# spartan-array/spartan

Measured on AMD Instinct MI355X. Metric: spartan.dot TFLOP/s (+ map/reduce HBM GB/s), higher is better.
Workload: dtype f32

## Files before the change

### spartan_amd/csrc/gemm_split.hpp

```cpp
#pragma once

typedef __bf16 gs_bf16x8 __attribute__((ext_vector_type(8)));
typedef __bf16 gs_bf16x4 __attribute__((ext_vector_type(4)));

namespace {

constexpr int GS_BK = 16;
constexpr int GS_RB = GS_BK * 2;
constexpr int GS_WN = 4;
constexpr unsigned GS_WIN_LO = (127u - 40u) << 23;
constexpr unsigned GS_WIN_HI = (127u + 40u) << 23;
constexpr size_t GS_IMAGE_CAP = (size_t)2 << 30;
constexpr size_t GS_WS_HEAD = 512;

template <int WN>
struct GsCfg {
  static constexpr int BM = 256, BN = 64 * WN, NW = 2 * WN, THREADS = 64 * NW;
  static constexpr int A_BYTES = BM * GS_RB, B_BYTES = BN * GS_RB;
  static constexpr int STAGE_BYTES = 3 * A_BYTES + 3 * B_BYTES;
  static constexpr int SMEM_BYTES = 2 * STAGE_BYTES;
  static constexpr int APW = A_BYTES / 1024 / NW, BPW = B_BYTES / 1024 / NW;
  static constexpr int NPIECES = 3 * APW + 3 * BPW;
  static constexpr int SLOTS = SP_CUS * (WN == 4 ? 1 : 2);
  static_assert(APW >= 1 && BPW >= 1 && APW * NW * 1024 == A_BYTES && BPW * NW * 1024 == B_BYTES, "tile / waves mismatch");
  static_assert(NPIECES * 4 <= 48, "one piece after every fourth MFMA");
};

__device__ __forceinline__ bool gs_outside(float v) {
  const unsigned b = __float_as_uint(v) & 0x7fffffffu;
  return b != 0u && (b < GS_WIN_LO || b >= GS_WIN_HI);
}

__device__ __forceinline__ void gs_cut(float v, __bf16& h, __bf16& m, __bf16& l) {
  h = (__bf16)v;
  const float r1 = v - (float)h;
  m = (__bf16)r1;
  l = (__bf16)(r1 - (float)m);
}

__device__ __forceinline__ void gs_raise(bool bad, unsigned* flag) {
  if (__any(bad) && (threadIdx.x & 63) == 0) atomicOr(flag, 1u);
}

__global__ __launch_bounds__(256) void sp_gemm_cut_rows_kernel(const float* __restrict__ A, int64_t lda, int M, int K,
                                                               __bf16* __restrict__ Ah, int64_t img,
                                                               unsigned* __restrict__ flag) {
  const int q = threadIdx.x & 7, row = blockIdx.x * 32 + (threadIdx.x >> 3);
  const int kpad = (K + GS_BK - 1) / GS_BK * GS_BK;
  bool bad = false;
  if (row < M) {
    const float* __restrict__ a = A + (int64_t)row * lda;
#pragma unroll
    for (int it = 0; it < 8; ++it) {
      const int k = blockIdx.y * 256 + it * 32 + 4 * q;
      if (k >= kpad) break;
      f32x4 v = {0.f, 0.f, 0.f, 0.f};
      if (k + 4 <= K) {
        v = *(const f32x4*)(a + k);
      } else {
#pragma unroll
        for (int e = 0; e < 4; ++e)
          if (k + e < K) v[e] = a[k + e];
      }
      gs_bf16x4 h, m, l;
#pragma unroll
      for (int e = 0; e < 4; ++e) {
        bad |= gs_outside(v[e]);
        __bf16 hh, mm, ll;
        gs_cut(v[e], hh, mm, ll);
        h[e] = hh;
        m[e] = mm;
        l[e] = ll;
      }
      const int64_t at = ((int64_t)(k >> 4) * M + row) * GS_BK + (k & 15);
      *(gs_bf16x4*)(Ah + at) = h;
      *(gs_bf16x4*)(Ah + img + at) = m;
      *(gs_bf16x4*)(Ah + 2 * img + at) = l;
    }
  }
  gs_raise(bad, flag);
}

__global__ __launch_bounds__(256) void sp_gemm_cut_cols_kernel(const float* __restrict__ B, int64_t ldb, int N, int K,
                                                               __bf16* __restrict__ Bh, int64_t img,
                                                               unsigned* __restrict__ flag) {
  __shared__ __attribute__((aligned(16))) __bf16 s[3][256 * GS_BK];
  const int n0 = blockIdx.x * 256, col = n0 + threadIdx.x, k0 = blockIdx.y * GS_BK;
  float v[GS_BK];
#pragma unroll
  for (int e = 0; e < GS_BK; ++e) v[e] = (col < N && k0 + e < K) ? B[(int64_t)(k0 + e) * ldb + col] : 0.f;
  bool bad = false;
  gs_bf16x8 h[2], m[2], l[2];
#pragma unroll
  for (int e = 0; e < GS_BK; ++e) {
    bad |= gs_outside(v[e]);
    __bf16 hh, mm, ll;
    gs_cut(v[e], hh, mm, ll);
    h[e >> 3][e & 7] = hh;
    m[e >> 3][e & 7] = mm;
    l[e >> 3][e & 7] = ll;
  }
#pragma unroll
  for (int c = 0; c < 2; ++c) {
    *(gs_bf16x8*)(&s[0][threadIdx.x * GS_BK + 8 * c]) = h[c];
    *(gs_bf16x8*)(&s[1][threadIdx.x * GS_BK + 8 * c]) = m[c];
    *(gs_bf16x8*)(&s[2][threadIdx.x * GS_BK + 8 * c]) = l[c];
  }
  __syncthreads();
  const int64_t base = ((int64_t)blockIdx.y * N + n0) * GS_BK;
#pragma unroll
  for (int p = 0; p < 3; ++p)
#pragma unroll
    for (int c = 0; c < 2; ++c) {
      const int at = (c * 256 + threadIdx.x) * 8;
      if (n0 + at / GS_BK < N) *(gs_bf16x8*)(Bh + p * img + base + at) = *(const gs_bf16x8*)(&s[p][at]);
    }
  gs_raise(bad, flag);
}

template <int WN>
__global__ __launch_bounds__(GsCfg<WN>::THREADS, 2) void sp_gemm_glds_kernel_bf16x3(
    const char* __restrict__ Ah, int64_t a_img, const char* __restrict__ Bh, int64_t b_img, float* __restrict__ C,
    int64_t ldc, int M, int N, int KT, int accumulate, int tiles_m, int tiles_n, int64_t a_slab, int64_t b_slab,
    const unsigned* __restrict__ flag_a, const unsigned* __restrict__ flag_b) {
  using G = GsCfg<WN>;
  constexpr int APW = G::APW, BPW = G::BPW, NPIECES = G::NPIECES;
  extern __shared__ __attribute__((aligned(16))) char gs_smem[];
  if ((*flag_a | *flag_b) != 0u) return;
  int tm, tn;
  sp_gemm_tile_of_block(blockIdx.x, gridDim.x, tiles_m, tiles_n, tm, tn);
  const int m0 = tm * G::BM, n0 = tn * G::BN;
  const int tid = threadIdx.x, lane = tid & 63;
  const int wid = __builtin_amdgcn_readfirstlane(tid >> 6);
  const int wm = wid / WN, wn = wid % WN;
  const int l31 = lane & 31, lh = lane >> 5;

  unsigned a_off[APW], b_off[BPW];
#pragma unroll
  for (int j = 0; j < APW; ++j) {
    const int slot = (wid * APW + j) * 64 + lane;
    int row = slot >> 1;
    const int q = (slot & 1) ^ ((row >> 4) & 1);
    if (m0 + row > M - 1) row = M - 1 - m0;
    a_off[j] = (unsigned)(row * GS_RB + q * 16);
  }
#pragma unroll
  for (int j = 0; j < BPW; ++j) {
    const int slot = (wid * BPW + j) * 64 + lane;
    int row = slot >> 1;
    const int q = (slot & 1) ^ ((row >> 4) & 1);
    if (n0 + row > N - 1) row = N - 1 - n0;
    b_off[j] = (unsigned)(row * GS_RB + q * 16);
  }
  const char* __restrict__ Ablk = Ah + (int64_t)m0 * GS_RB;
  const char* __restrict__ Bblk = Bh + (int64_t)n0 * GS_RB;
  const unsigned s_base = SP_LDS_ADDR(gs_smem);

#define GS_PIECE(i)                                                                                    \
  do {                                                                                                 \
    if ((i) < 3 * APW) {                                                                               \
      const int p_ = (i) / APW, j_ = (i) % APW;                                                        \
      SP_GLDS_S(Ablk + p_ * a_img + ka_, a_off[j_], st_ + p_ * G::A_BYTES + (wid * APW + j_) * 1024);  \
    } else {                                                                                           \
      const int p_ = ((i) - 3 * APW) / BPW, j_ = ((i) - 3 * APW) % BPW;                                \
      SP_GLDS_S(Bblk + p_ * b_img + kb_, b_off[j_],                                                    \
                st_ + 3 * G::A_BYTES + p_ * G::B_BYTES + (wid * BPW + j_) * 1024);                     \
    }                                                                                                  \
  } while (0)

  f32x16 acc[4][2];
#pragma unroll
  for (int i = 0; i < 4; ++i)
#pragma unroll
    for (int j = 0; j < 2; ++j)
#pragma unroll
      for (int r = 0; r < 16; ++r) acc[i][j][r] = 0.f;

  {
    const int64_t ka_ = 0, kb_ = 0;
    const unsigned st_ = s_base;
#pragma unroll
    for (int i = 0; i < NPIECES; ++i) GS_PIECE(i);
  }
  SP_GLDS_LANDED();
  __syncthreads();

  const int fslot = (lh ^ ((l31 >> 4) & 1)) * 16;
  const int a_frag = (wm * 128 + l31) * GS_RB + fslot;
  const int b_frag = 3 * G::A_BYTES + (wn * 64 + l31) * GS_RB + fslot;

  for (int t = 0; t < KT; ++t) {
    const bool more = t + 1 < KT;
    const int64_t ka_ = (int64_t)(t + 1) * a_slab, kb_ = (int64_t)(t + 1) * b_slab;
    const unsigned st_ = s_base + (unsigned)((t + 1) & 1) * G::STAGE_BYTES;
    const char* st = gs_smem + (t & 1) * G::STAGE_BYTES;
    gs_bf16x8 af[3][4], bf[3][2];
#pragma unroll
    for (int p = 0; p < 3; ++p) {
#pragma unroll
      for (int i = 0; i < 4; ++i) af[p][i] = *(const gs_bf16x8*)(st + p * G::A_BYTES + a_frag + i * 32 * GS_RB);
#pragma unroll
      for (int j = 0; j < 2; ++j) bf[p][j] = *(const gs_bf16x8*)(st + p * G::B_BYTES + b_frag + j * 32 * GS_RB);
    }
    int piece = 0;
#pragma unroll
    for (int idx = 0; idx < 48; ++idx) {
      const int term = idx >> 3, i = (idx & 7) >> 1, j = idx & 1;
      const int pa = term == 0 ? 2 : (term == 2 || term == 3) ? 1 : 0;
      const int pb = term == 1 ? 2 : (term == 2 || term == 4) ? 1 : 0;
      acc[i][j] = __builtin_amdgcn_mfma_f32_32x32x16_bf16(af[pa][i], bf[pb][j], acc[i][j], 0, 0, 0);
      if (idx % 4 == 3 && piece < NPIECES) {
        __builtin_amdgcn_sched_barrier(0);
        if (more) GS_PIECE(piece);
        __builtin_amdgcn_sched_barrier(0);
        ++piece;
      }
    }
    if (more) SP_GLDS_LANDED();
    __syncthreads();
  }
#undef GS_PIECE

#pragma unroll
  for (int i = 0; i < 4; ++i) {
#pragma unroll
    for (int j = 0; j < 2; ++j) {
      const int col = n0 + wn * 64 + j * 32 + l31;
#pragma unroll
      for (int r = 0; r < 16; ++r) {
        const int row = m0 + wm * 128 + i * 32 + (r & 3) + 8 * (r >> 2) + 4 * lh;
        if (row < M && col < N) {
          float* p = C + (int64_t)row * ldc + col;
          float v = acc[i][j][r];
          if (accumulate) v += *p;
          *p = v;
        }
      }
    }
  }
}

template <typename Cfg, int BM, int BN, int WM, int WN, int WGS>
__global__ __launch_bounds__(Cfg::THREADS, WGS) void sp_gemm_f32_gated_kernel(
    const float* __restrict__ A, int64_t lda, const float* __restrict__ B, int64_t ldb, float* __restrict__ C,
    int64_t ldc, int M, int N, int K, int accumulate, int tiles_m, int tiles_n, const unsigned* __restrict__ flag_a,
    const unsigned* __restrict__ flag_b) {
  if ((*flag_a | *flag_b) == 0u) return;
  sp_gemm_glds_body<Cfg, BM, BN, WM, WN>(A, lda, B, ldb, C, ldc, M, N, K, accumulate, tiles_m, tiles_n);
}

#define GS_CUT_BYTES_PER_S 3.0e12
#define GS_ISSUED_FLOPS 1.1e15
static bool sp_gemm_bf16_plan(int64_t M, int64_t N, int64_t K) {
  static int mode = -2;
  if (mode == -2) {
    const char* e = getenv("SP_GEMM_SPLIT");
    mode = e ? atoi(e) : 1;
  }
  using G = GsCfg<GS_WN>;
  if (mode == 0 || K < 16 || N % 4 != 0 || N < 4 || M < 1 || M > 2147483647LL || N > 2147483647LL || K > 2147483647LL)
    return false;
  const int64_t tb = ((M + 255) / 256) * ((N + 127) / 128);
  if (tb < 2 * SP_CUS || tb >= 2147483647LL) return false;
  double dp_cost;
  if (sp_gemm_dp_choice(M, N, &dp_cost) != 6 || sp_sk_plan(M, N, K)) return false;
  const int64_t KT = (K + GS_BK - 1) / GS_BK;
  if ((double)KT * 3.0 * GS_RB * ((double)M + (double)N) > (double)GS_IMAGE_CAP) return false;
  const double fp32_s = dp_cost * 128.0 * 128.0 * (double)K * 2.0 / (157.3e12 * 0.95 / SP_CUS);
  const int64_t tiles = ((M + G::BM - 1) / G::BM) * ((N + G::BN - 1) / G::BN);
  const int64_t rounds = (tiles + G::SLOTS - 1) / G::SLOTS;
  const double main_s = (double)rounds * G::SLOTS * (6.0 * 2.0 * G::BM * G::BN * (double)K) / GS_ISSUED_FLOPS;
  const double cut_s = 10.0 * ((double)M + (double)N) * (double)K / GS_CUT_BYTES_PER_S;
  return (main_s + cut_s + 20e-6) < 0.92 * fp32_s;
}

static size_t sp_gemm_bf16_ws_bytes(int64_t M, int64_t N, int64_t K) {
  return GS_WS_HEAD + (size_t)((K + GS_BK - 1) / GS_BK) * 3 * GS_RB * (size_t)(M + N);
}

constexpr size_t GS_IMG_HEAD = 256;

static size_t sp_gemm_bf16_image_bytes(int64_t rows, int64_t K) {
  return GS_IMG_HEAD + (size_t)((K + GS_BK - 1) / GS_BK) * 3 * GS_RB * (size_t)rows;
}

static long long gs_cut_launches = 0;

static void sp_gemm_bf16_cut(int side, const float* X, int64_t ld, int64_t rows, int64_t K, char* img, unsigned* flag,
                             hipStream_t st) {
  const int64_t KT = (K + GS_BK - 1) / GS_BK;
  const int64_t img_stride = KT * rows * GS_RB;
  __atomic_add_fetch(&gs_cut_launches, 1, __ATOMIC_RELAXED);
  if (side == 0)
    hipLaunchKernelGGL(sp_gemm_cut_rows_kernel, dim3((unsigned)((rows + 31) / 32), (unsigned)((K + 255) / 256)), dim3(256), 0,
                       st, X, ld, (int)rows, (int)K, (__bf16*)img, img_stride / 2, flag);
  else
    hipLaunchKernelGGL(sp_gemm_cut_cols_kernel, dim3((unsigned)((rows + 255) / 256), (unsigned)KT), dim3(256), 0, st, X, ld,
                       (int)rows, (int)K, (__bf16*)img, img_stride / 2, flag);
}

static int sp_gemm_bf16_launch(const float* A, int64_t lda, const char* imgA, int64_t a_rows, int64_t a_row0,
                               const float* B, int64_t ldb, const char* imgB, int64_t b_rows, int64_t b_row0, float* C,
                               int64_t ldc, int64_t M, int64_t N, int64_t K, int acc, void* ws, hipStream_t st) {
  using G = GsCfg<GS_WN>;
  const int64_t KT = (K + GS_BK - 1) / GS_BK;
  const int64_t tiles_m = (M + G::BM - 1) / G::BM, tiles_n = (N + G::BN - 1) / G::BN;
  auto kern = sp_gemm_glds_kernel_bf16x3<GS_WN>;
  using FCfg = GldsCfg<256, 128, 2, 2>;
  auto gated = sp_gemm_f32_gated_kernel<FCfg, 256, 128, 2, 2, 2>;
  static bool attr_set = false;
  if (!attr_set) {
    SP_HIP(hipFuncSetAttribute((const void*)kern, hipFuncAttributeMaxDynamicSharedMemorySize, G::SMEM_BYTES));
    SP_HIP(hipFuncSetAttribute((const void*)gated, hipFuncAttributeMaxDynamicSharedMemorySize, FCfg::LDS_BYTES));
    attr_set = true;
  }
  char* base = (char*)(((uintptr_t)ws + 255) & ~(uintptr_t)255);
  char* next = base + GS_IMG_HEAD;
  if (!imgA || !imgB) SP_HIP(hipMemsetAsync(base, 0, GS_IMG_HEAD, st));
  const unsigned* flag_a = (const unsigned*)(imgA ? imgA : base);
  const unsigned* flag_b = (const unsigned*)(imgB ? imgB : base);
  const char *Ah, *Bh;
  if (imgA) {
    Ah = imgA + GS_IMG_HEAD + a_row0 * GS_RB;
  } else {
    a_rows = M;
    sp_gemm_bf16_cut(0, A, lda, M, K, next, (unsigned*)base, st);
    Ah = next;
    next += 3 * KT * M * GS_RB;
  }
  if (imgB) {
    Bh = imgB + GS_IMG_HEAD + b_row0 * GS_RB;
  } else {
    b_rows = N;
    sp_gemm_bf16_cut(1, B, ldb, N, K, next, (unsigned*)base, st);
    Bh = next;
  }
  hipLaunchKernelGGL(kern, dim3((unsigned)(tiles_m * tiles_n)), dim3(G::THREADS), G::SMEM_BYTES, st, Ah,
                     KT * a_rows * GS_RB, Bh, KT * b_rows * GS_RB, C, ldc, (int)M, (int)N, (int)KT, acc, (int)tiles_m,
                     (int)tiles_n, a_rows * GS_RB, b_rows * GS_RB, flag_a, flag_b);
  const int64_t ftm = (M + 255) / 256, ftn = (N + 127) / 128;
  hipLaunchKernelGGL(gated, dim3((unsigned)(ftm * ftn)), dim3(FCfg::THREADS), FCfg::LDS_BYTES, st, A, lda, B, ldb, C, ldc,
                     (int)M, (int)N, (int)K, acc, (int)ftm, (int)ftn, flag_a, flag_b);
  SP_CHECK_LAUNCH();
  return 0;
}

}
```

Before: 257.6.

## Software-pipeline LDS fragment reads with MFMAs and prefetch two k-tiles ahead

```diff
diff --git a/spartan_amd/csrc/gemm_split.hpp b/spartan_amd/csrc/gemm_split.hpp
--- a/spartan_amd/csrc/gemm_split.hpp
+++ b/spartan_amd/csrc/gemm_split.hpp
@@ -24,6 +24,11 @@
   static constexpr int SLOTS = SP_CUS * (WN == 4 ? 1 : 2);
   static_assert(APW >= 1 && BPW >= 1 && APW * NW * 1024 == A_BYTES && BPW * NW * 1024 == B_BYTES, "tile / waves mismatch");
   static_assert(NPIECES * 4 <= 48, "one piece after every fourth MFMA");
+};
+
+template <int V>
+struct GsInt {
+  static constexpr int value = V;
 };
 
 __device__ __forceinline__ bool gs_outside(float v) {
@@ -176,6 +181,60 @@
 #pragma unroll
       for (int r = 0; r < 16; ++r) acc[i][j][r] = 0.f;
 
+  const int fslot = (lh ^ ((l31 >> 4) & 1)) * 16;
+  const int a_frag = (wm * 128 + l31) * GS_RB + fslot;
+  const int b_frag = 3 * G::A_BYTES + (wn * 64 + l31) * GS_RB + fslot;
+  const unsigned a_rd[2] = {s_base + (unsigned)a_frag, s_base + (unsigned)(G::STAGE_BYTES + a_frag)};
+  const unsigned b_rd[2] = {s_base + (unsigned)b_frag, s_base + (unsigned)(G::STAGE_BYTES + b_frag)};
+
+  gs_bf16x8 am[4], al[4], bm[2], bl[2], ah[2][4], bh[2][2];
+#define GS_READ_A(dst, s_, p_, i_) \
+  asm volatile("ds_read_b128 %0, %1 offset:%2" : "+v"(dst) : "v"(a_rd[s_]), "n"((p_) * G::A_BYTES + (i_) * 32 * GS_RB) : "memory")
+#define GS_READ_B(dst, s_, p_, j_) \
+  asm volatile("ds_read_b128 %0, %1 offset:%2" : "+v"(dst) : "v"(b_rd[s_]), "n"((p_) * G::B_BYTES + (j_) * 32 * GS_RB) : "memory")
+#define GS_READS_DONE(s_)                                                                                             \
+  do {                                                                                                                \
+    asm volatile("s_waitcnt lgkmcnt(0)"                                                                               \
+                 : "+v"(al[0]), "+v"(al[1]), "+v"(al[2]), "+v"(al[3]), "+v"(am[0]), "+v"(am[1]), "+v"(am[2]),          \
+                   "+v"(am[3]), "+v"(bl[0]), "+v"(bl[1]), "+v"(bm[0]), "+v"(bm[1])                                     \
+                 :: "memory");                                                                                        \
+    asm volatile("" : "+v"(ah[s_][0]), "+v"(ah[s_][1]), "+v"(ah[s_][2]), "+v"(ah[s_][3]), "+v"(bh[s_][0]),             \
+                      "+v"(bh[s_][1]) :: "memory");                                                                   \
+  } while (0)
+
+  auto ktile = [&](auto par_, const bool rd, const bool ld, int t) __attribute__((always_inline)) {
+    constexpr int CUR = decltype(par_)::value, NXT = CUR ^ 1;
+    const int64_t ka_ = (int64_t)(t + 2) * a_slab, kb_ = (int64_t)(t + 2) * b_slab;
+    const unsigned st_ = s_base + (unsigned)CUR * G::STAGE_BYTES;
+#pragma unroll
+    for (int idx = 0; idx < 48; ++idx) {
+      const int term = idx >> 3, i = (idx & 7) >> 1, j = idx & 1;
+      const gs_bf16x8 a = term == 0 ? al[i] : (term == 2 || term == 3) ? am[i] : ah[CUR][i];
+      const gs_bf16x8 b = term == 1 ? bl[j] : (term == 2 || term == 4) ? bm[j] : bh[CUR][j];
+      acc[i][j] = __builtin_amdgcn_mfma_f32_32x32x16_bf16(a, b, acc[i][j], 0, 0, 0);
+      __builtin_amdgcn_sched_barrier(0);
+      if (rd) {
+        const int q = idx & 7, r = q < 3 ? q : q - 1;
+        if (term == 0 && q != 3 && q != 7) {
+          if (r < 4) GS_READ_A(ah[NXT][r & 3], NXT, 0, r & 3);
+          else GS_READ_B(bh[NXT][r & 1], NXT, 0, r & 1);
+        }
+        if (term == 1 && q != 3 && r < 4) GS_READ_A(al[r & 3], NXT, 2, r & 3);
+        if (term == 2 && q < 2) GS_READ_B(bl[q & 1], NXT, 2, q & 1);
+        if (term == 4 && q < 4) GS_READ_A(am[q & 3], NXT, 1, q & 3);
+        if (term == 5 && q < 2) GS_READ_B(bm[q & 1], NXT, 1, q & 1);
+      }
+      if (ld && idx % 4 == 3 && idx / 4 < NPIECES) GS_PIECE(idx / 4);
+      __builtin_amdgcn_sched_barrier(0);
+    }
+    if (ld) SP_GLDS_LANDED();
+    if (rd) GS_READS_DONE(NXT);
+    __syncthreads();
+    __builtin_amdgcn_sched_barrier(0);
+  };
+  GsInt<0> even;
+  GsInt<1> odd;
+
   {
     const int64_t ka_ = 0, kb_ = 0;
     const unsigned st_ = s_base;
@@ -184,41 +243,39 @@
   }
   SP_GLDS_LANDED();
   __syncthreads();
-
-  const int fslot = (lh ^ ((l31 >> 4) & 1)) * 16;
-  const int a_frag = (wm * 128 + l31) * GS_RB + fslot;
-  const int b_frag = 3 * G::A_BYTES + (wn * 64 + l31) * GS_RB + fslot;
-
-  for (int t = 0; t < KT; ++t) {
-    const bool more = t + 1 < KT;
-    const int64_t ka_ = (int64_t)(t + 1) * a_slab, kb_ = (int64_t)(t + 1) * b_slab;
-    const unsigned st_ = s_base + (unsigned)((t + 1) & 1) * G::STAGE_BYTES;
-    const char* st = gs_smem + (t & 1) * G::STAGE_BYTES;
-    gs_bf16x8 af[3][4], bf[3][2];
-#pragma unroll
-    for (int p = 0; p < 3; ++p) {
-#pragma unroll
-      for (int i = 0; i < 4; ++i) af[p][i] = *(const gs_bf16x8*)(st + p * G::A_BYTES + a_frag + i * 32 * GS_RB);
-#pragma unroll
-      for (int j = 0; j < 2; ++j) bf[p][j] = *(const gs_bf16x8*)(st + p * G::B_BYTES + b_frag + j * 32 * GS_RB);
-    }
-    int piece = 0;
-#pragma unroll
-    for (int idx = 0; idx < 48; ++idx) {
-      const int term = idx >> 3, i = (idx & 7) >> 1, j = idx & 1;
-      const int pa = term == 0 ? 2 : (term == 2 || term == 3) ? 1 : 0;
-      const int pb = term == 1 ? 2 : (term == 2 || term == 4) ? 1 : 0;
-      acc[i][j] = __builtin_amdgcn_mfma_f32_32x32x16_bf16(af[pa][i], bf[pb][j], acc[i][j], 0, 0, 0);
-      if (idx % 4 == 3 && piece < NPIECES) {
-        __builtin_amdgcn_sched_barrier(0);
-        if (more) GS_PIECE(piece);
-        __builtin_amdgcn_sched_barrier(0);
-        ++piece;
-      }
-    }
-    if (more) SP_GLDS_LANDED();
-    __syncthreads();
-  }
+  if (KT > 1) {
+    const int64_t ka_ = a_slab, kb_ = b_slab;
+    const unsigned st_ = s_base + G::STAGE_BYTES;
+#pragma unroll
+    for (int i = 0; i < NPIECES; ++i) GS_PIECE(i);
+  }
+#pragma unroll
+  for (int i = 0; i < 4; ++i) {
+    ah[0][i] = ah[1][i] = am[i] = al[i] = gs_bf16x8{};
+    GS_READ_A(ah[0][i], 0, 0, i);
+    GS_READ_A(am[i], 0, 1, i);
+    GS_READ_A(al[i], 0, 2, i);
+  }
+#pragma unroll
+  for (int j = 0; j < 2; ++j) {
+    bh[0][j] = bh[1][j] = bm[j] = bl[j] = gs_bf16x8{};
+    GS_READ_B(bh[0][j], 0, 0, j);
+    GS_READ_B(bm[j], 0, 1, j);
+    GS_READ_B(bl[j], 0, 2, j);
+  }
+  SP_GLDS_LANDED();
+  GS_READS_DONE(0);
+  __syncthreads();
+
+  int t = 0;
+  for (; t + 1 < KT; t += 2) {
+    ktile(even, true, t + 2 < KT, t);
+    ktile(odd, t + 2 < KT, t + 3 < KT, t + 1);
+  }
+  if (t < KT) ktile(even, false, false, t);
+#undef GS_READ_A
+#undef GS_READ_B
+#undef GS_READS_DONE
 #undef GS_PIECE
 
 #pragma unroll
```

Result: faster. 265.0, median of 6 (+2.9%).
